# Andy-ckm/K8S-GPU-

Hardware: AMD Instinct MI355X
Metric: p50 reconcile-to-Ready latency (s) + readyReplicas accuracy at replicas=1/2/4/8 (lower is better)
Workload: dtype bf16

## Files before the change

gpupool/ops/probe.py:

```python
from __future__ import annotations

import ctypes
import functools
import json
import threading

from . import lowp, native_path

_lib = None
_lock = threading.Lock()
_count: int | None = None


def lib() -> ctypes.CDLL:
    global _lib
    with _lock:
        if _lib is None:
            l = ctypes.CDLL(native_path("libmi355x_probe.so"))
            l.mi355x_probe_init.restype = ctypes.c_int
            l.mi355x_probe_init.argtypes = [ctypes.c_char_p, ctypes.c_size_t]
            l.mi355x_probe_device_count.restype = ctypes.c_int
            l.mi355x_probe_identify.restype = ctypes.c_void_p
            l.mi355x_probe_identify.argtypes = [ctypes.c_int]
            l.mi355x_probe_run.restype = ctypes.c_void_p
# ... 3 lines not shown
            l.mi355x_probe_peer.argtypes = [ctypes.c_int, ctypes.c_int, ctypes.c_char_p]
            if hasattr(l, "mi355x_probe_peer_ring"):
                l.mi355x_probe_peer_ring.restype = ctypes.c_void_p
                l.mi355x_probe_peer_ring.argtypes = [ctypes.POINTER(ctypes.c_int), ctypes.c_int,
                                                     ctypes.c_char_p]
            l.mi355x_probe_trim.restype = ctypes.c_int
            l.mi355x_probe_trim.argtypes = [ctypes.c_int]
            l.mi355x_probe_hbm_sweep.restype = ctypes.c_void_p
            l.mi355x_probe_hbm_sweep.argtypes = [ctypes.c_int, ctypes.c_char_p]
            l.mi355x_probe_sweep_alloc.restype = ctypes.c_int
            l.mi355x_probe_sweep_alloc.argtypes = [ctypes.c_int, ctypes.c_longlong]
            l.mi355x_probe_sweep_release.restype = ctypes.c_int
            l.mi355x_probe_sweep_release.argtypes = [ctypes.c_int]
            l.mi355x_probe_gemm_bf16.restype = ctypes.c_int
            l.mi355x_probe_gemm_bf16.argtypes = [ctypes.c_int, ctypes.c_void_p, ctypes.c_void_p,
                                                 ctypes.c_void_p, ctypes.c_int, ctypes.c_int,
                                                 ctypes.c_int]
            if hasattr(l, "mi355x_probe_gemm_bf16_opts"):
                l.mi355x_probe_gemm_bf16_opts.restype = ctypes.c_int
                l.mi355x_probe_gemm_bf16_opts.argtypes = [ctypes.c_int, ctypes.c_void_p,
                                                          ctypes.c_void_p, ctypes.c_void_p,
                                                          ctypes.c_int, ctypes.c_int, ctypes.c_int,
                                                          ctypes.c_char_p]
            if hasattr(l, "mi355x_probe_gemm_lowp"):
                l.mi355x_probe_gemm_lowp.restype = ctypes.c_int
                l.mi355x_probe_gemm_lowp.argtypes = [ctypes.c_int, ctypes.c_int] + [ctypes.c_void_p] * 5 + \
                    [ctypes.c_int] * 3 + [ctypes.c_char_p]
            if hasattr(l, "mi355x_probe_host_link"):
                l.mi355x_probe_host_link.restype = ctypes.c_void_p
                l.mi355x_probe_host_link.argtypes = [ctypes.c_int, ctypes.c_char_p, ctypes.c_void_p,
                                                     ctypes.c_size_t]
                l.mi355x_probe_host_link_geometry.restype = None
                l.mi355x_probe_host_link_geometry.argtypes = [ctypes.POINTER(ctypes.c_int)] * 3
            if hasattr(l, "mi355x_probe_lds"):
                l.mi355x_probe_lds.restype = ctypes.c_void_p
                l.mi355x_probe_lds.argtypes = [ctypes.c_int, ctypes.c_char_p, ctypes.c_void_p, ctypes.c_size_t]
            if hasattr(l, "mi355x_probe_abft_check"):
                vp, ull = ctypes.c_void_p, ctypes.c_ulonglong
                l.mi355x_probe_abft_check.restype = ctypes.c_int
                l.mi355x_probe_abft_check.argtypes = [ctypes.c_int, ctypes.c_int] + [vp] * 5 + \
                    [ctypes.c_int] * 3 + [ctypes.c_float, vp, vp, ctypes.c_int, vp, vp, vp]
                l.mi355x_probe_gemm_ref.restype = ctypes.c_int
                l.mi355x_probe_gemm_ref.argtypes = [ctypes.c_int, ctypes.c_int] + [vp] * 5 + [ctypes.c_int] * 3
                l.mi355x_probe_count_diff.restype = ctypes.c_int
                l.mi355x_probe_count_diff.argtypes = [ctypes.c_int, vp, vp, ull, ctypes.POINTER(ull)]
                l.mi355x_probe_gen_operands.restype = ctypes.c_int
                l.mi355x_probe_gen_operands.argtypes = [ctypes.c_int, ctypes.c_int, ctypes.c_uint, ctypes.c_int,
                                                        ull, ull, vp, ctypes.c_size_t, vp, ctypes.c_size_t,
                                                        vp, ctypes.c_size_t]
            _lib = l
    return _lib


def _take(p) -> dict:
    if not p:
        raise RuntimeError("libmi355x_probe returned NULL")
    try:
        return json.loads(ctypes.string_at(p).decode())
    finally:
        lib().mi355x_probe_free(p)


def init() -> int:
    global _count
    if _count is not None:
        return _count
# ... 9 lines not shown
    return _take(lib().mi355x_probe_identify(dev))


def run(dev: int, hbm_bytes: int = 1 << 30, mfma: bool = True, gemm_n: int = 4096,
        patterns: int = 2, gemm_reps: int = 1, gemm_tile: int = 256, mfma_low_precision=(),
        host_link_bytes: int = 0, lds_check: bool = False, **test_hooks: int) -> dict:
    opts = _run_opts(int(hbm_bytes), bool(mfma), int(gemm_n), int(patterns), int(gemm_reps),
                     int(gemm_tile), tuple(sorted((k, int(v)) for k, v in test_hooks.items())),
                     tuple(mfma_low_precision), int(host_link_bytes), bool(lds_check))
    return _take(lib().mi355x_probe_run(dev, opts))


@functools.lru_cache(maxsize=64)
def _run_opts(hbm_bytes: int, mfma: bool, gemm_n: int, patterns: int, gemm_reps: int,
              gemm_tile: int, hooks: tuple, low_precision: tuple = (),
              host_link_bytes: int = 0, lds_check: bool = False) -> bytes:
    opts = {"hbmBytes": hbm_bytes, "mfma": mfma, "gemmN": gemm_n, "patterns": patterns,
            "gemmReps": gemm_reps, "gemmTile": gemm_tile, **dict(hooks)}
    if low_precision:
        opts["mfmaLowPrecision"] = lowp.dtype_mask(low_precision)
    if host_link_bytes > 0:
        opts["hostLinkBytes"] = host_link_bytes
    if lds_check:
        opts["ldsCheck"] = 1
    return json.dumps(opts).encode()


def host_link_geometry() -> dict:
    if not hasattr(lib(), "mi355x_probe_host_link"):
        raise RuntimeError("libmi355x_probe.so predates the host-link check: rebuild it")
    g, t, u = ctypes.c_int(), ctypes.c_int(), ctypes.c_int()
    lib().mi355x_probe_host_link_geometry(ctypes.byref(g), ctypes.byref(t), ctypes.byref(u))
    return {"grid": g.value, "threads": t.value, "unroll": u.value}


def host_link(dev: int, nbytes: int, patterns: int = 2, preload=None, want_bytes: int = 0,
              **hooks: int) -> dict:
    if not hasattr(lib(), "mi355x_probe_host_link"):
        raise RuntimeError("libmi355x_probe.so predates the host-link check: rebuild it")
    opts = {"hostLinkBytes": int(nbytes), "hostLinkPatterns": int(patterns),
            **{k: int(v) for k, v in hooks.items()}}
    buf, n = None, 0
    if preload is not None:
        raw = bytes(preload) if not hasattr(preload, "tobytes") else preload.tobytes()
        n = len(raw)
        buf = ctypes.create_string_buffer(raw, n)
        opts["preload"] = 1
    elif want_bytes > 0:
        n = int(want_bytes)
        buf = ctypes.create_string_buffer(n)
    res = _take(lib().mi355x_probe_host_link(dev, json.dumps(opts).encode(), buf, n))
    if buf is not None and want_bytes > 0 and "bytes" in res:
        res["data"] = buf.raw[:min(int(want_bytes), n, int(res["bytes"]))]
    return res


def lds(dev: int, nbytes: int = 163840, patterns: int = 2, want_stage: int = 0, **hooks: int) -> dict:
    if not hasattr(lib(), "mi355x_probe_lds"):
        raise RuntimeError("libmi355x_probe.so predates the LDS check: rebuild it")
    opts = {"ldsBytes": int(nbytes), "ldsPatterns": int(patterns), **{k: int(v) for k, v in hooks.items()}}
    buf, n = None, 0
    if want_stage:
        opts["ldsDumpStage"] = int(want_stage)
        n = 163840
        buf = ctypes.create_string_buffer(n)
    res = _take(lib().mi355x_probe_lds(dev, json.dumps(opts).encode(), buf, n))
# ... 135 lines not shown
```

native/include/mi355x/probe.h:

```cpp
#ifndef MI355X_PROBE_H_
#define MI355X_PROBE_H_

#include <stddef.h>

#ifdef __cplusplus
extern "C" {
#endif

int mi355x_probe_init(char* err, size_t errlen);
int mi355x_probe_device_count(void);
char* mi355x_probe_identify(int device);
char* mi355x_probe_run(int device, const char* opts_json);
char* mi355x_probe_lds(int device, const char* opts_json, void* image, size_t image_bytes);
char* mi355x_probe_host_link(int device, const char* opts_json, void* io, size_t io_bytes);
void mi355x_probe_host_link_geometry(int* grid, int* threads, int* unroll);
char* mi355x_probe_peer(int src, int dst, const char* opts_json);
char* mi355x_probe_peer_ring(const int* devs, int n, const char* opts_json);
char* mi355x_probe_hbm_sweep(int device, const char* opts_json);
int mi355x_probe_sweep_alloc(int device, long long reserve_bytes);
int mi355x_probe_sweep_release(int device);
int mi355x_probe_gemm_bf16(int device, const void* A, const void* Bt, void* C, int m, int n, int k);
int mi355x_probe_gemm_bf16_opts(int device, const void* A, const void* Bt, void* C, int m, int n, int k,
                                const char* opts_json);
int mi355x_probe_gemm_lowp(int device, int dtype, const void* A, const void* Bt, const void* scaleA,
                           const void* scaleBt, void* C, int m, int n, int k, const char* opts_json);
int mi355x_probe_abft_check(int device, int dtype, const void* A, const void* Bt, const void* scaleA,
                            const void* scaleBt, const void* C, int m, int n, int k, float bound,
                            unsigned int* vectors, unsigned long long* counts, int nfaults,
                            const long long* fault_index, const float* fault_value,
                            unsigned long long* fault_counts);
int mi355x_probe_gemm_ref(int device, int dtype, const void* A, const void* Bt, const void* scaleA,
                          const void* scaleBt, void* R, int m, int n, int k);
int mi355x_probe_count_diff(int device, const float* x, const float* y, unsigned long long count,
                            unsigned long long* bad);
int mi355x_probe_gen_operands(int device, int dtype, unsigned int seed, int span_or_scale_lo,
                              unsigned long long count, unsigned long long nzero, void* operand,
                              size_t operand_bytes, void* scales, size_t scale_bytes, void* zero,
                              size_t zero_bytes);
void mi355x_probe_free(char* p);

#ifdef __cplusplus
}
#endif

#endif
```

native/src/probe/ctx.h:

```cpp
#pragma once

#include <chrono>
#include <cstdio>
#include <cstdlib>
#include <cstring>
#include <mutex>
#include <string>
#include <vector>

#include "arena.h"
#include "options.h"
#include "types.h"

namespace {

struct SweepBuf {
  std::vector<void*> chunks;
  uint64_t span = 0;
  bool empty() const { return chunks.empty(); }
};

struct DeviceCtx {
  hipStream_t stream = nullptr;
  hipStream_t stream2 = nullptr;
  hipEvent_t ev[1 + 2 * kMaxPatterns] = {};
  hipEvent_t gev[3] = {};
  hipDeviceProp_t prop{};
  unsigned long long* host_res = nullptr;
  hipEvent_t lev[lowp::kDtypes][2] = {};
  unsigned long long* host_lowp = nullptr;
  hipStream_t hl_stream = nullptr;
  hipEvent_t hev[1 + 2 * kMaxPatterns] = {};
  void* hl_buf = nullptr;
  void* hl_dev = nullptr;
  uint64_t hl_bytes = 0;
  bool hl_coherent = true;
  unsigned long long* hl_cnt = nullptr;
  unsigned long long* hl_res = nullptr;
  hipEvent_t lds_ev[2] = {};
  unsigned long long* lds_cnt = nullptr;
  unsigned long long* lds_res = nullptr;
  int lds_set = 0;
  bool lds_clean = false;
  uint32_t lds_runs = 0;
  void* lds_dump = nullptr;
  void* arena = nullptr;
  size_t arena_bytes = 0;
  std::chrono::steady_clock::time_point arena_used{};
  SweepBuf sweep;
  unsigned long long* sweep_cnt = nullptr;
  std::chrono::steady_clock::time_point sweep_released{};
  void* peer_send = nullptr;
  void* peer_recv = nullptr;
  uint64_t peer_bytes = 0;
  unsigned long long* peer_cnt = nullptr;
  std::chrono::steady_clock::time_point peer_used{};
  std::string uuid;
  bool ready = false;
};

constexpr std::chrono::seconds kSweepClearGrace{30};
// ... 17 lines not shown
struct DevBuf {
  void* p = nullptr;
  ~DevBuf() {
    if (p) (void)hipFree(p);
  }
};

inline std::string hip_uuid(int dev) {
  hipUUID u{};
  if (hipDeviceGetUuid(&u, dev) != hipSuccess) return "";
  std::string s(u.bytes, u.bytes + 16);
  bool ascii = true;
  for (char c : s) ascii = ascii && ((c >= '0' && c <= '9') || (c >= 'a' && c <= 'f') || (c >= 'A' && c <= 'F'));
  if (ascii) return "GPU-" + s;
  char buf[40];
  std::string hex;
  for (int i = 0; i < 16; ++i) {
    std::snprintf(buf, sizeof buf, "%02x", static_cast<unsigned char>(u.bytes[i]));
    hex += buf;
  }
  return "GPU-" + hex;
}

inline DeviceCtx& ensure_ctx(int dev) {
  PROBE_CHECK(hipSetDevice(dev));
  DeviceCtx& ctx = ctx_of(dev);
  if (ctx.ready) return ctx;
  PROBE_CHECK(hipStreamCreateWithFlags(&ctx.stream, hipStreamNonBlocking));
  PROBE_CHECK(hipStreamCreateWithFlags(&ctx.stream2, hipStreamNonBlocking));
  for (auto& e : ctx.ev) PROBE_CHECK(hipEventCreate(&e));
  for (auto& e : ctx.gev) PROBE_CHECK(hipEventCreate(&e));
  PROBE_CHECK(hipGetDeviceProperties(&ctx.prop, dev));
  PROBE_CHECK(hipHostMalloc(reinterpret_cast<void**>(&ctx.host_res), kResSlots * sizeof(unsigned long long)));
  ctx.uuid = hip_uuid(dev);
  ctx.ready = true;
  return ctx;
}

}
```

native/src/probe/hbm.h:

```cpp
#pragma once

#include <algorithm>
#include <cstdint>

#include "options.h"
#include "report.h"
#include "types.h"

namespace {

__host__ __device__ __forceinline__ uint32_t pattern_word(uint64_t idx, uint32_t seed) {
  uint32_t x = static_cast<uint32_t>(idx) * 0x9E3779B1u ^ static_cast<uint32_t>(idx >> 32) * 0x85EBCA77u;
  x ^= seed;
  x ^= x >> 15;
  x *= 0x2C1B3C6Du;
  x ^= x >> 12;
  return x;
}

template <int kPat>
__host__ __device__ __forceinline__ u32x4 pattern16(uint64_t i16, uint32_t seed, uint32_t flip) {
  u32x4 v;
  if constexpr (kPat == 0) {
    uint64_t w = i16 * 4;
    v.x = pattern_word(w, seed) ^ flip;
    v.y = pattern_word(w + 1, seed) ^ flip;
    v.z = pattern_word(w + 2, seed) ^ flip;
    v.w = pattern_word(w + 3, seed) ^ flip;
  } else {
    uint32_t h = (static_cast<uint32_t>(i16) ^ seed) * 0x9E3779B1u;
    h ^= __builtin_rotateleft32(static_cast<uint32_t>(i16 >> 32), 7);
    h ^= h >> 15;
    v.x = h ^ flip;
    v.y = __builtin_rotateleft32(h, 8) ^ 0xA5A5A5A5u ^ flip;
    v.z = __builtin_rotateleft32(h, 16) ^ 0x3C96C396u ^ flip;
    v.w = __builtin_rotateleft32(h, 24) ^ 0x5A0FF05Au ^ flip;
  }
  return v;
}
__device__ __forceinline__ uint64_t umin64(uint64_t a, uint64_t b) { return a < b ? a : b; }

constexpr int kHbmThreads = 256;
constexpr int kHbmUnroll = 4;

constexpr uint64_t kHbmTile = static_cast<uint64_t>(kHbmThreads) * kHbmUnroll;

__device__ __forceinline__ void reset_pairs(unsigned long long* __restrict__ cnt, int nreset) {
  if (blockIdx.x == 0 && static_cast<int>(threadIdx.x) < 2 * nreset)
    cnt[threadIdx.x] = (threadIdx.x & 1) ? ~0ull : 0ull;
}

template <int kPat = kHbmPattern, int kLayout = 0>
__global__ __launch_bounds__(kHbmThreads) void hbm_fill(u32x4* __restrict__ p, uint64_t n16,
                                                        uint32_t seed, uint32_t flip,
                                                        unsigned long long* __restrict__ reset, int nreset) {
  reset_pairs(reset, nreset);
  const uint64_t stride = static_cast<uint64_t>(gridDim.x) * kHbmThreads;
  if constexpr (kLayout == 1) {
    const uint64_t tiles = n16 / kHbmTile;
    for (uint64_t t = blockIdx.x; t < tiles; t += gridDim.x) {
      const uint64_t base = t * kHbmTile + threadIdx.x;
#pragma unroll
      for (int u = 0; u < kHbmUnroll; ++u) {
        const uint64_t j = base + static_cast<uint64_t>(u) * kHbmThreads;
        __builtin_nontemporal_store(pattern16<kPat>(j, seed, flip), &p[j]);
      }
    }
    for (uint64_t i = tiles * kHbmTile + static_cast<uint64_t>(blockIdx.x) * kHbmThreads + threadIdx.x; i < n16;
         i += stride)
      __builtin_nontemporal_store(pattern16<kPat>(i, seed, flip), &p[i]);
    return;
  }
  uint64_t i = static_cast<uint64_t>(blockIdx.x) * kHbmThreads + threadIdx.x;
  for (; i + (kHbmUnroll - 1) * stride < n16; i += kHbmUnroll * stride) {
#pragma unroll
    for (int u = 0; u < kHbmUnroll; ++u) {
      uint64_t j = i + u * stride;
      __builtin_nontemporal_store(pattern16<kPat>(j, seed, flip), &p[j]);
    }
  }
  for (; i < n16; i += stride) __builtin_nontemporal_store(pattern16<kPat>(i, seed, flip), &p[i]);
}

__device__ __forceinline__ uint32_t mismatches16(u32x4 v, u32x4 e) {
  return __builtin_popcount(v.x ^ e.x) + __builtin_popcount(v.y ^ e.y) +
         __builtin_popcount(v.z ^ e.z) + __builtin_popcount(v.w ^ e.w);
}

template <int kPat = kHbmPattern, int kLayout = 0>
__global__ __launch_bounds__(kHbmThreads) void hbm_verify(const u32x4* __restrict__ p, uint64_t n16,
                                                          uint32_t seed, uint32_t flip,
                                                          unsigned long long* __restrict__ bad_bits,
                                                          unsigned long long* __restrict__ first_bad) {
  const uint64_t stride = static_cast<uint64_t>(gridDim.x) * kHbmThreads;
  uint32_t bad = 0;
  uint64_t first = ~0ull;
  auto check = [&](u32x4 v, uint64_t j) {
    uint32_t m = mismatches16(v, pattern16<kPat>(j, seed, flip));
    if (m) {
      bad += m;
      first = umin64(first, j);
    }
  };
  if constexpr (kLayout == 1) {
    const uint64_t tiles = n16 / kHbmTile;
    for (uint64_t t = blockIdx.x; t < tiles; t += gridDim.x) {
      const uint64_t base = t * kHbmTile + threadIdx.x;
      u32x4 v[kHbmUnroll];
#pragma unroll
      for (int u = 0; u < kHbmUnroll; ++u) v[u] = __builtin_nontemporal_load(&p[base + static_cast<uint64_t>(u) * kHbmThreads]);
#pragma unroll
      for (int u = 0; u < kHbmUnroll; ++u) check(v[u], base + static_cast<uint64_t>(u) * kHbmThreads);
    }
    for (uint64_t i = tiles * kHbmTile + static_cast<uint64_t>(blockIdx.x) * kHbmThreads + threadIdx.x; i < n16;
         i += stride)
      check(__builtin_nontemporal_load(&p[i]), i);
  } else {
    uint64_t i = static_cast<uint64_t>(blockIdx.x) * kHbmThreads + threadIdx.x;
    for (; i + (kHbmUnroll - 1) * stride < n16; i += kHbmUnroll * stride) {
      u32x4 v[kHbmUnroll];
#pragma unroll
      for (int u = 0; u < kHbmUnroll; ++u) v[u] = __builtin_nontemporal_load(&p[i + u * stride]);
#pragma unroll
      for (int u = 0; u < kHbmUnroll; ++u) check(v[u], i + u * stride);
    }
    for (; i < n16; i += stride) check(__builtin_nontemporal_load(&p[i]), i);
  }
#pragma unroll
  for (int off = 32; off > 0; off >>= 1) {
    bad += __shfl_xor(bad, off, 64);
    first = umin64(first, static_cast<uint64_t>(__shfl_xor(static_cast<unsigned long long>(first), off, 64)));
  }
  if ((threadIdx.x & 63) == 0 && bad) {
    atomicAdd(bad_bits, static_cast<unsigned long long>(bad));
    atomicMin(first_bad, static_cast<unsigned long long>(first));
  }
}
__global__ void inject_bit_flips(unsigned int* __restrict__ p, uint64_t nwords, int count) {
  const uint64_t stride = nwords / static_cast<uint64_t>(count + 1);
  for (int i = threadIdx.x; i < count; i += blockDim.x) p[static_cast<uint64_t>(i + 1) * stride] ^= 1u << (i % 32);
}

static_assert(2 * kMaxPatterns <= kHbmThreads, "hbm_fill resets the HBM pairs from one block");

inline int hbm_grid(int cus, long long per_cu, uint64_t n16) {
  return static_cast<int>(std::min<uint64_t>(static_cast<uint64_t>(cus) * static_cast<uint64_t>(per_cu),
                                             (n16 + kHbmThreads - 1) / kHbmThreads));
}

inline void memset_pairs(hipStream_t s, unsigned long long* cnt, int zero_words, int npairs) {
  PROBE_CHECK(hipMemsetAsync(cnt, 0, zero_words * sizeof(unsigned long long), s));
  for (int pi = 0; pi < npairs; ++pi)
    PROBE_CHECK(hipMemsetAsync(cnt + 2 * pi + 1, 0xFF, sizeof(unsigned long long), s));
}

struct PatternPass {
  hipStream_t s = nullptr;
  u32x4* buf = nullptr;
  uint64_t n16 = 0;
  uint32_t seed = 0;
  int fill_grid = 1, verify_grid = 1;
  bool cheap = kHbmPattern == 1, tiled = false;

  static uint32_t flip_of(int pi) { return (pi & 1) ? 0xFFFFFFFFu : 0u; }

  void fill(int pi, unsigned long long* reset = nullptr, int nreset = 0) const {
    const dim3 grid(fill_grid), block(kHbmThreads);
    if (tiled) hipLaunchKernelGGL((hbm_fill<1, 1>), grid, block, 0, s, buf, n16, seed, flip_of(pi), reset, nreset);
    else if (cheap) hipLaunchKernelGGL(hbm_fill<1>, grid, block, 0, s, buf, n16, seed, flip_of(pi), reset, nreset);
    else hipLaunchKernelGGL(hbm_fill<0>, grid, block, 0, s, buf, n16, seed, flip_of(pi), reset, nreset);
  }

  void verify(int pi, unsigned long long* pair) const {
    const dim3 grid(verify_grid), block(kHbmThreads);
    const u32x4* p = buf;
    if (tiled) hipLaunchKernelGGL((hbm_verify<1, 1>), grid, block, 0, s, p, n16, seed, flip_of(pi), pair, pair + 1);
    else if (cheap) hipLaunchKernelGGL(hbm_verify<1>, grid, block, 0, s, p, n16, seed, flip_of(pi), pair, pair + 1);
    else hipLaunchKernelGGL(hbm_verify<0>, grid, block, 0, s, p, n16, seed, flip_of(pi), pair, pair + 1);
  }

  void inject_flips(int count) const {
    hipLaunchKernelGGL(inject_bit_flips, dim3(1), dim3(256), 0, s, reinterpret_cast<unsigned int*>(buf), n16 * 4, count);
  }
  void inject_flip_at(uint64_t chunk) const {
    hipLaunchKernelGGL(inject_bit_flips, dim3(1), dim3(256), 0, s, reinterpret_cast<unsigned int*>(buf + chunk),
                       uint64_t{0}, 1);
  }
};

inline void fold_pairs(const unsigned long long* pairs, int patterns, HbmResult* r) {
  for (int pi = 0; pi < patterns; ++pi) {
    r->bad_bits += pairs[2 * pi];
    r->first_bad = std::min(r->first_bad, pairs[2 * pi + 1]);
  }
}

inline HbmResult fold_passes(const hipEvent_t* ev, const unsigned long long* pairs, int patterns, uint64_t n16) {
  HbmResult r;
  r.n16 = n16;
  r.patterns = patterns;
  for (int pi = 0; pi < patterns; ++pi) {
    float w, rd;
    PROBE_CHECK(hipEventElapsedTime(&w, ev[2 * pi], ev[1 + 2 * pi]));
    PROBE_CHECK(hipEventElapsedTime(&rd, ev[1 + 2 * pi], ev[2 + 2 * pi]));
    r.write_ms += w;
    r.read_ms += rd;
  }
  fold_pairs(pairs, patterns, &r);
  return r;
}

// ... 2 lines not shown
```

native/src/probe/options.h:

```cpp
#pragma once

#include <algorithm>
#include <cstdint>
#include <cstdlib>
#include <cstring>
#include <stdexcept>
#include <string>

namespace {

inline long long opt_int(const char* json, const char* key, long long def) {
  if (!json) return def;
  std::string pat = std::string("\"") + key + "\"";
  const char* p = std::strstr(json, pat.c_str());
  if (!p) return def;
  p = std::strchr(p + pat.size(), ':');
  if (!p) return def;
  ++p;
  while (*p == ' ') ++p;
  if (std::strncmp(p, "true", 4) == 0) return 1;
  if (std::strncmp(p, "false", 5) == 0) return 0;
  return std::strtoll(p, nullptr, 10);
}

inline bool opt_bool(const char* json, const char* key, bool def) { return opt_int(json, key, def) != 0; }

constexpr long long kMaxPatterns = 4;

constexpr int kHbmPattern = 1;
constexpr int kHbmLayout = 0;
constexpr long long kHbmFillBlocksPerCU = 1, kHbmVerifyBlocksPerCU = 3;

constexpr int kGemmGroupM = 4;
constexpr int kGemmPipe = 2;

struct GemmVariant {
  int tile = 256;
  int pipe = kGemmPipe;
  bool prio = false;
  bool vec_c = false;
};

struct GemmOptions {
  GemmVariant variant;
  int group_m = kGemmGroupM;
  bool poison_c = false;
  static GemmOptions parse(const char* json) {
    GemmOptions o;
    o.variant.tile = static_cast<int>(opt_int(json, "gemmTile", 256));
    o.variant.pipe = static_cast<int>(opt_int(json, "gemmPipe", kGemmPipe));
    o.variant.prio = opt_bool(json, "gemmPrio", false);
    o.variant.vec_c = opt_bool(json, "gemmVecC", false);
    o.group_m = static_cast<int>(opt_int(json, "gemmGroupM", kGemmGroupM));
    o.poison_c = opt_bool(json, "poisonC", false);
    return o;
  }
};

namespace lowp {
enum Dtype { kFp8 = 0, kMxFp8 = 1, kMxFp4 = 2, kDtypes = 3 };
constexpr const char* kNames[kDtypes] = {"fp8", "mxfp8", "mxfp4"};
}

// ... 72 lines not shown
    pl.n16 = static_cast<uint32_t>(bytes / 16);
    pl.patterns = static_cast<int>(std::min(kMaxPatterns, std::max(1LL, opt_int(json, "ldsPatterns", 2))));
    const long long salt = opt_int(json, "ldsSalt", -1);
    pl.salt_given = salt >= 0;
    pl.salt = pl.salt_given ? static_cast<uint32_t>(salt) : 0u;
    pl.seed = 0x4C445300u + static_cast<uint32_t>(dev);
    pl.blocks_per_cu =
        static_cast<int>(std::min<long long>(kMaxBlocksPerCU, std::max(1LL, opt_int(json, "ldsBlocksPerCU", kBlocksPerCU))));
    pl.flip_byte = opt_int(json, "injectLdsFlipAtByte", -1);
    pl.fault_xcc = static_cast<int>(opt_int(json, "injectLdsFaultXcc", -1));
    pl.skip_chunk = opt_int(json, "injectLdsSkipChunk", -1);
    const long long stage = opt_int(json, "ldsDumpStage", 0);
    pl.dump_stage = stage >= 1 && stage <= 3 ? static_cast<int>(stage) : 0;
    return pl;
  }
};

}

struct FaultAt {
  long long row = -1, col = -1;
  long long index(int n) const {
    const long long r = row == -1 ? n / 3 : row, c = col == -1 ? n / 5 : col;
    if (r < 0 || r >= n || c < 0 || c >= n) return -1;
    return r * n + c;
  }
};

struct ProbeOptions {
  uint64_t hbm_bytes = 1ull << 30;
  int patterns = 2;
  bool cheap_pattern = true;
  bool tiled = false;
  long long fill_blocks_per_cu = kHbmFillBlocksPerCU;
  long long verify_blocks_per_cu = kHbmVerifyBlocksPerCU;
  int inject_flips = 0;
  long long inject_chunk = -1;
  bool mfma = true;
  int gemm_n = 4096;
  GemmOptions gemm;
  int reps = 1;
  int inject_gemm = 0;
  FaultAt inject_gemm_at;
  int census_fault_xcc = -1;
  bool require_all_cus = true;
  bool cu_keys = false;
  int lowp_mask = 0;
  int inject_lowp = 0;
  int lowp_census_fault_xcc = -1;
  bool overlap = true;
  int hbm_first = 1;
  bool zero_in_kernel = true;
  bool keep_arena = true;
  hostlink::Plan host_link;
  bool host_link_on_mfma_stream = false;
  lds::Plan lds;
  bool lds_first = lds::kFirst == 1;

  static ProbeOptions parse(const char* json, int dev = 0) {
    ProbeOptions o;
    o.hbm_bytes = static_cast<uint64_t>(opt_int(json, "hbmBytes", 1LL << 30));
    o.patterns = static_cast<int>(std::min(kMaxPatterns, std::max(1LL, opt_int(json, "patterns", 2))));
    o.cheap_pattern = opt_int(json, "hbmPattern", kHbmPattern) == 1;
    o.tiled = o.cheap_pattern && opt_int(json, "hbmLayout", kHbmLayout) == 1;
    o.fill_blocks_per_cu =
        std::max(1LL, opt_int(json, "hbmFillBlocksPerCU", opt_int(json, "hbmBlocksPerCU", kHbmFillBlocksPerCU)));
    o.verify_blocks_per_cu =
        std::max(1LL, opt_int(json, "hbmVerifyBlocksPerCU", opt_int(json, "hbmBlocksPerCU", kHbmVerifyBlocksPerCU)));
    o.inject_flips = static_cast<int>(std::min(4096LL, std::max(0LL, opt_int(json, "injectBitFlips", 0))));
    o.inject_chunk = opt_int(json, "injectFlipAtChunk", -1);
    o.mfma = opt_bool(json, "mfma", true);
    o.gemm_n = std::max(256, (static_cast<int>(opt_int(json, "gemmN", 4096)) / 256) * 256);
    o.gemm = GemmOptions::parse(json);
    o.gemm.variant.tile = o.gemm.variant.tile != 128 ? 256 : 128;
    o.reps = opt_int(json, "gemmSkip", 0) ? 0 : static_cast<int>(std::max(1LL, opt_int(json, "gemmReps", 1)));
    o.inject_gemm = static_cast<int>(opt_int(json, "injectGemmFault", 0));
    o.inject_gemm_at.row = opt_int(json, "injectGemmFaultRow", -1);
    o.inject_gemm_at.col = opt_int(json, "injectGemmFaultCol", -1);
    o.census_fault_xcc = static_cast<int>(opt_int(json, "injectCensusFaultXcc", -1));
    o.require_all_cus = opt_bool(json, "requireAllCUs", true);
    o.cu_keys = opt_bool(json, "cuKeys", false);
    o.lowp_mask = o.mfma ? static_cast<int>(opt_int(json, "mfmaLowPrecision", 0)) & ((1 << lowp::kDtypes) - 1) : 0;
    o.inject_lowp = static_cast<int>(opt_int(json, "injectLowpFault", 0));
    o.lowp_census_fault_xcc = static_cast<int>(opt_int(json, "injectLowpCensusFaultXcc", -1));
    o.overlap = opt_bool(json, "overlap", true);
    o.hbm_first = static_cast<int>(opt_int(json, "hbmFirst", 1));
    o.zero_in_kernel = opt_bool(json, "zeroInKernel", true);
    o.keep_arena = opt_bool(json, "keepArena", true);
    const uint64_t hl_bytes = static_cast<uint64_t>(std::max(0LL, opt_int(json, "hostLinkBytes", 0)));
    if (hl_bytes > hostlink::kMaxBytes) throw std::invalid_argument("hostLinkBytes above 4 GiB");
    if (hl_bytes) {
      o.host_link = hostlink::Plan::parse(json, dev, hl_bytes);
      o.host_link_on_mfma_stream = o.overlap && opt_int(json, "hostLinkStream", 0) == 1;
    }
    if (opt_bool(json, "ldsCheck", false)) {
      o.lds = lds::Plan::parse(json, dev);
      o.lds.dump_stage = 0;
      o.lds_first = opt_int(json, "ldsFirst", lds::kFirst) == 1;
    }
    return o;
  }
};

struct HostLinkOptions {
  bool preload = false;
  uint64_t bytes = 0;
  static HostLinkOptions parse(const char* json) {
    HostLinkOptions o;
    o.preload = opt_bool(json, "preload", false);
    o.bytes = static_cast<uint64_t>(std::max(0LL, opt_int(json, "hostLinkBytes", 0)));
    return o;
  }
};

inline uint64_t peer_bytes(const char* json, long long def) {
  return static_cast<uint64_t>(std::max(1LL << 20, opt_int(json, "bytes", def)));
}

struct SweepOptions {
  uint64_t bytes = 16ull << 30;
  uint64_t reserve = 4ull << 30;
// ... 16 lines not shown
```

native/src/probe/probe.hip:

```cpp
#include <hip/hip_runtime.h>

#include <algorithm>
#include <chrono>
#include <cstdlib>
#include <cstring>
#include <mutex>
#include <string>
#include <vector>

#include "mi355x/probe.h"

#include "arena.h"
#include "ctx.h"
#include "hbm.h"
#include "hostlink.h"
#include "lds.h"
#include "lowp.h"
#include "mfma_phase.h"
#include "options.h"
#include "peer.h"
#include "report.h"
#include "sweep.h"
#include "types.h"

// ... 44 lines not shown
  memset_pairs(s, cnt, kResSlots, o.patterns);
  if (o.overlap) {
    PROBE_CHECK(hipEventRecord(ctx.gev[2], s));
    PROBE_CHECK(hipStreamWaitEvent(s2, ctx.gev[2], 0));
  }
}

lowp::Phase lowp_phase(DeviceCtx& ctx, const ProbeOptions& o, char* base, const ArenaLayout& lay) {
  lowp::Phase lp;
  lp.mask = o.lowp_mask;
  lp.region = base + lay.lowp_region;
  lp.cnt = reinterpret_cast<unsigned long long*>(base + lay.lowp_cnt);
  lp.host = ctx.host_lowp;
  lp.ev = ctx.lev;
  lp.gemm_n = o.gemm_n;
  lp.cus = ctx.prop.multiProcessorCount;
  lp.inject_mask = o.inject_lowp;
  lp.inject_at = o.inject_gemm_at.index(o.gemm_n);
  lp.census_fault_xcc = o.lowp_census_fault_xcc;
  lp.poison_c = o.gemm.poison_c;
  return lp;
}

PatternPass hbm_pass(DeviceCtx& ctx, const ProbeOptions& o, int dev, char* base, const ArenaLayout& lay, uint64_t n16) {
  PatternPass pass;
  pass.s = ctx.stream;
  pass.buf = reinterpret_cast<u32x4*>(base + lay.hbm);
  pass.n16 = n16;
  pass.seed = 0xA5A50000u + static_cast<uint32_t>(dev);
  pass.fill_grid = hbm_grid(ctx.prop.multiProcessorCount, o.fill_blocks_per_cu, n16);
  pass.verify_grid = hbm_grid(ctx.prop.multiProcessorCount, o.verify_blocks_per_cu, n16);
  pass.cheap = o.cheap_pattern;
  pass.tiled = o.tiled;
  return pass;
}

template <class F>
void enqueue_hbm(DeviceCtx& ctx, const PatternPass& pass, const ProbeOptions& o, unsigned long long* cnt,
                 F&& after_first_fill) {
  PROBE_CHECK(hipEventRecord(ctx.ev[0], pass.s));
  for (int pi = 0; pi < o.patterns; ++pi) {
    unsigned long long* reset = o.zero_in_kernel && pi == 0 ? cnt : nullptr;
    pass.fill(pi, reset, reset ? o.patterns : 0);
    PROBE_CHECK(hipEventRecord(ctx.ev[1 + 2 * pi], pass.s));
    if (pi == 0) {
      after_first_fill();
      if (o.inject_flips > 0) pass.inject_flips(o.inject_flips);
      if (o.inject_chunk >= 0 && static_cast<uint64_t>(o.inject_chunk) < pass.n16)
        pass.inject_flip_at(static_cast<uint64_t>(o.inject_chunk));
    }
    pass.verify(pi, cnt + 2 * pi);
    PROBE_CHECK(hipEventRecord(ctx.ev[2 + 2 * pi], pass.s));
  }
  PROBE_CHECK(hipGetLastError());
  PROBE_CHECK(hipMemcpyAsync(ctx.host_res, cnt, 2 * o.patterns * sizeof(unsigned long long), hipMemcpyDeviceToHost, pass.s));
}

std::string run_probe(int dev, const char* opts) {
  const ProbeOptions o = ProbeOptions::parse(opts, dev);
  auto t0 = std::chrono::steady_clock::now();
  DeviceCtx& ctx = ensure_ctx(dev);
  if (o.lowp_mask) ensure_lowp(ctx);
  hostlink::Plan hl = o.host_link;
  hipStream_t s = ctx.stream, s2 = o.overlap ? ctx.stream2 : s, hl_s = s;
  if (hl.n16) {
    hl.alloc_ms = hostlink::ensure(ctx, hl.n16 * 16, hl.coherent);
// ... 8 lines not shown

  auto t_alloc = std::chrono::steady_clock::now();
  const uint64_t n16 = o.hbm_bytes / 16;
  const ArenaLayout lay = ArenaLayout::make(n16, o.gemm_n, o.mfma, o.lowp_mask);
  DevBuf transient;
  char* base = acquire_arena(ctx, lay.need, o.keep_arena, &transient, &t.arena_reused);
  auto* cnt = reinterpret_cast<unsigned long long*>(base + lay.cnt);
  t.alloc_ms = ms_since(t_alloc);

  auto t_run = std::chrono::steady_clock::now();
  reset_counters(ctx, o, cnt, s, s2);
  const lowp::Phase lp = lowp_phase(ctx, o, base, lay);
  bool lds_pending = ld.n16 != 0;
  auto enqueue_lds = [&](bool here) {
    if (!lds_pending || !here) return;
    lds::launch(ctx, s2, ld);
    lds_pending = false;
  };
  auto enqueue_mfma = [&](int when) {
    if (!o.mfma || o.hbm_first != when) return;
    enqueue_lds(o.overlap && o.lds_first);
    launch_mfma_phase(base, lay, o, ctx, s2);
    lowp::launch(s2, lp);
    enqueue_lds(o.overlap);
  };
  const PatternPass pass = hbm_pass(ctx, o, dev, base, lay, n16);
  enqueue_mfma(0);
  enqueue_hbm(ctx, pass, o, cnt, [&] { enqueue_mfma(2); });
  enqueue_mfma(1);
  enqueue_lds(true);
  if (hl.n16) hostlink::launch(ctx, hl_s, hl);
  t.launch_ms = ms_since(t_run);

  PROBE_CHECK(hipStreamSynchronize(s));
  t.hbm_wall_ms = ms_since(t_run);
  rep.mfma.enabled = o.mfma;
  rep.mfma.n = o.gemm_n;
  rep.mfma.tile = o.gemm.variant.tile;
  rep.mfma.pipe = o.gemm.variant.tile == 256 ? o.gemm.variant.pipe : 0;
  if (o.mfma) {
    PROBE_CHECK(hipStreamSynchronize(s2));
    finish_mfma(o, ctx, &rep.mfma, &rep.cus);
  }
  rep.has_lds = ld.n16 != 0;
  if (ld.n16) {
    if (!o.mfma && s2 != s) PROBE_CHECK(hipStreamSynchronize(s2));
    rep.lds = lds::finish(ctx, ld, o.require_all_cus);
  }
  rep.lowp = lowp::finish(lp, o.require_all_cus);
  t.mfma_wall_ms = o.mfma ? ms_since(t_run) : 0.0;
  rep.has_host_link = hl.n16 != 0;
  if (hl.n16) {
    if (hl_s != s && !(hl_s == ctx.stream2 && o.mfma)) PROBE_CHECK(hipStreamSynchronize(hl_s));
    rep.host_link = hostlink::finish(ctx, hl);
  }
  rep.hbm = fold_passes(ctx.ev, ctx.host_res, o.patterns, n16);
  auto t_free = std::chrono::steady_clock::now();
  if (transient.p) {
    (void)hipFree(transient.p);
    transient.p = nullptr;
  }
  t.free_ms = ms_since(t_free);
  rep.total_ms = ms_since(t0);

  const auto t_report = std::chrono::steady_clock::now();
  rep.dev = dev;
  rep.uuid = ctx.uuid;
  rep.arch = ctx.prop.gcnArchName;
  std::string out = probe_report_open(rep);
  out += ",\"reportMs\":" + jnum(ms_since(t_report)) + "}";
  return out;
}

template <class F>
char* guarded(const std::string& head, F&& body) {
  try {
    return dup(body());
  } catch (const std::exception& e) {
    (void)hipGetLastError();
    return dup(error_report(head, e.what()));
  }
}

// ... 362 lines not shown
    need = count * 2;
  } else {
    if (count % (32 / lowp::bits_of(dtype)) || nzero || zero || span_or_scale_lo < -126 || span_or_scale_lo > 126) return -2;
    need = count * lowp::bits_of(dtype) / 8;
  }
  if (operand_bytes < need || (has_scales ? (!scales || scale_bytes < count / 32) : scales != nullptr)) return -2;
  if (zero ? zero_bytes < nzero * 4 : nzero > 0) return -2;
  std::lock_guard<std::mutex> g(device_mutex(dev));
  return guarded_status([&] {
    PROBE_CHECK(hipSetDevice(dev));
    DevBuf dop, dsc, dz;
    auto filled = [](DevBuf& d, size_t bytes) {
      PROBE_CHECK(hipMalloc(&d.p, std::max<size_t>(bytes, 16)));
      PROBE_CHECK(hipMemset(d.p, 0xFF, std::max<size_t>(bytes, 16)));
    };
    filled(dop, operand_bytes);
    if (has_scales) filled(dsc, scale_bytes);
    if (zero) filled(dz, zero_bytes);
    launch_generator(nullptr, dtype, dop.p, count, static_cast<uint8_t*>(dsc.p), seed, span_or_scale_lo,
                     static_cast<uint32_t*>(dz.p), nzero);
    PROBE_CHECK(hipGetLastError());
    PROBE_CHECK(hipMemcpy(operand, dop.p, operand_bytes, hipMemcpyDeviceToHost));
    if (has_scales && scale_bytes) PROBE_CHECK(hipMemcpy(scales, dsc.p, scale_bytes, hipMemcpyDeviceToHost));
    if (zero && zero_bytes) PROBE_CHECK(hipMemcpy(zero, dz.p, zero_bytes, hipMemcpyDeviceToHost));
  });
}

void mi355x_probe_host_link_geometry(int* grid, int* threads, int* unroll) {
  if (grid) *grid = hostlink::kGrid;
  if (threads) *threads = hostlink::kThreads;
  if (unroll) *unroll = hostlink::kUnroll;
}

char* mi355x_probe_host_link(int dev, const char* opts_json, void* io, size_t io_bytes) {
  if (!device_ok(dev)) return bad_device();
  const HostLinkOptions o = HostLinkOptions::parse(opts_json);
  if (o.preload && !io) return dup(error_report("", "preload needs a caller buffer"));
  ProbeActive active;
  std::lock_guard<std::mutex> g(device_mutex(dev));
  return guarded(device_head(dev), [&] {
    DeviceCtx& ctx = ensure_ctx(dev);
    const uint64_t bytes = o.preload ? static_cast<uint64_t>(io_bytes) : o.bytes;
    if (bytes < 16 || bytes > hostlink::kMaxBytes) throw ProbeError("host-link size outside [16 B, 4 GiB]");
    hostlink::Plan pl = hostlink::Plan::parse(opts_json, dev, bytes);
    if (o.preload) {
      pl.preload = true;
      pl.patterns = 1;
    }
    pl.alloc_ms = hostlink::ensure(ctx, pl.n16 * 16, pl.coherent);
    if (o.preload) std::memcpy(ctx.hl_buf, io, pl.n16 * 16);
    hostlink::launch(ctx, ctx.stream, pl);
    PROBE_CHECK(hipStreamSynchronize(ctx.stream));
    const HostLinkResult r = hostlink::finish(ctx, pl);
    if (io) std::memcpy(io, ctx.hl_buf, std::min<uint64_t>(io_bytes, pl.n16 * 16));
    return "{" + device_head(dev) + ",\"passed\":" + jbool(r.ok()) + "," + host_link_block(r).substr(1);
  });
}

int mi355x_probe_gemm_bf16(int dev, const void* A, const void* Bt, void* C, int m, int n, int k) {
  return mi355x_probe_gemm_bf16_opts(dev, A, Bt, C, m, n, k, nullptr);
}

char* mi355x_probe_lds(int dev, const char* opts_json, void* image, size_t image_bytes) {
  if (!device_ok(dev)) return bad_device();
  ProbeActive active;
  std::lock_guard<std::mutex> g(device_mutex(dev));
// ... 19 lines not shown
```

Before: 0.005100.

## Add atomic work-claiming tail layout to HBM fill/verify and fold side streams first

Adds a new HBM layout, made the default, where each block strides through a static head region and then takes row units of the remaining tail through a global atomic counter. The aim is to balance load across blocks and stop the slowest CU from setting the finish time of the fill and verify passes. It also changes the host ordering so results from the side streams (MFMA, LDS) are synchronized and folded before the wait on the main HBM stream, overlapping that host work. The costs are per-block atomics, per-pass counter resets that chain kernels through a `next` pointer, and added geometry bookkeeping with bounds checks in the tail.

```diff
diff --git a/gpupool/ops/probe.py b/gpupool/ops/probe.py
--- a/gpupool/ops/probe.py
+++ b/gpupool/ops/probe.py
@@ -59,6 +59,11 @@
                                                      ctypes.c_size_t]
                 l.mi355x_probe_host_link_geometry.restype = None
                 l.mi355x_probe_host_link_geometry.argtypes = [ctypes.POINTER(ctypes.c_int)] * 3
+            if hasattr(l, "mi355x_probe_hbm_claim_geometry"):
+                ullp = ctypes.POINTER(ctypes.c_ulonglong)
+                l.mi355x_probe_hbm_claim_geometry.restype = ctypes.c_int
+                l.mi355x_probe_hbm_claim_geometry.argtypes = [ctypes.c_int, ctypes.c_ulonglong, ctypes.c_int, ullp, ullp,
+                                                              ctypes.POINTER(ctypes.c_uint), ullp]
             if hasattr(l, "mi355x_probe_lds"):
                 l.mi355x_probe_lds.restype = ctypes.c_void_p
                 l.mi355x_probe_lds.argtypes = [ctypes.c_int, ctypes.c_char_p, ctypes.c_void_p, ctypes.c_size_t]
@@ -134,6 +139,17 @@
     g, t, u = ctypes.c_int(), ctypes.c_int(), ctypes.c_int()
     lib().mi355x_probe_host_link_geometry(ctypes.byref(g), ctypes.byref(t), ctypes.byref(u))
     return {"grid": g.value, "threads": t.value, "unroll": u.value}
+
+
+def hbm_claim_geometry(dev: int, nbytes: int, verify: bool = False) -> dict:
+    if not hasattr(lib(), "mi355x_probe_hbm_claim_geometry"):
+        raise RuntimeError("libmi355x_probe.so predates the claimed HBM layout: rebuild it")
+    head, units, width, rows = ctypes.c_ulonglong(), ctypes.c_ulonglong(), ctypes.c_ulonglong(), ctypes.c_uint()
+    rc = lib().mi355x_probe_hbm_claim_geometry(dev, int(nbytes), int(bool(verify)), ctypes.byref(head),
+                                               ctypes.byref(units), ctypes.byref(rows), ctypes.byref(width))
+    if rc != 0:
+        raise RuntimeError(f"mi355x_probe_hbm_claim_geometry failed (rc={rc})")
+    return {"head": head.value, "units": units.value, "unitRows": rows.value, "rowWidth": width.value}
 
 
 def host_link(dev: int, nbytes: int, patterns: int = 2, preload=None, want_bytes: int = 0,
diff --git a/native/include/mi355x/probe.h b/native/include/mi355x/probe.h
--- a/native/include/mi355x/probe.h
+++ b/native/include/mi355x/probe.h
@@ -14,6 +14,9 @@
 char* mi355x_probe_lds(int device, const char* opts_json, void* image, size_t image_bytes);
 char* mi355x_probe_host_link(int device, const char* opts_json, void* io, size_t io_bytes);
 void mi355x_probe_host_link_geometry(int* grid, int* threads, int* unroll);
+int mi355x_probe_hbm_claim_geometry(int device, unsigned long long bytes, int verify, unsigned long long* head,
+                                    unsigned long long* units, unsigned int* unit_rows,
+                                    unsigned long long* row_width);
 char* mi355x_probe_peer(int src, int dst, const char* opts_json);
 char* mi355x_probe_peer_ring(const int* devs, int n, const char* opts_json);
 char* mi355x_probe_hbm_sweep(int device, const char* opts_json);
diff --git a/native/src/probe/ctx.h b/native/src/probe/ctx.h
--- a/native/src/probe/ctx.h
+++ b/native/src/probe/ctx.h
@@ -27,6 +27,8 @@
   hipEvent_t gev[3] = {};
   hipDeviceProp_t prop{};
   unsigned long long* host_res = nullptr;
+  unsigned int* hbm_claims = nullptr;
+  bool hbm_claims_clean = false;
   hipEvent_t lev[lowp::kDtypes][2] = {};
   unsigned long long* host_lowp = nullptr;
   hipStream_t hl_stream = nullptr;
@@ -110,6 +112,9 @@
   for (auto& e : ctx.gev) PROBE_CHECK(hipEventCreate(&e));
   PROBE_CHECK(hipGetDeviceProperties(&ctx.prop, dev));
   PROBE_CHECK(hipHostMalloc(reinterpret_cast<void**>(&ctx.host_res), kResSlots * sizeof(unsigned long long)));
+  PROBE_CHECK(hipMalloc(reinterpret_cast<void**>(&ctx.hbm_claims), 2 * kMaxPatterns * sizeof(unsigned int)));
+  PROBE_CHECK(hipMemsetAsync(ctx.hbm_claims, 0, 2 * kMaxPatterns * sizeof(unsigned int), ctx.stream));
+  ctx.hbm_claims_clean = true;
   ctx.uuid = hip_uuid(dev);
   ctx.ready = true;
   return ctx;
diff --git a/native/src/probe/hbm.h b/native/src/probe/hbm.h
--- a/native/src/probe/hbm.h
+++ b/native/src/probe/hbm.h
@@ -3,6 +3,7 @@
 #include <algorithm>
 #include <cstdint>
 
+#include "hbm_claims.h"
 #include "options.h"
 #include "report.h"
 #include "types.h"
@@ -44,6 +45,41 @@
 constexpr int kHbmUnroll = 4;
 
 constexpr uint64_t kHbmTile = static_cast<uint64_t>(kHbmThreads) * kHbmUnroll;
+static_assert(kHbmThreads == kHbmClaimColumn && kHbmUnroll == kHbmClaimUnroll, "hbm_claims.h describes these kernels");
+
+struct HbmClaims {
+  unsigned int* counter = nullptr;
+  unsigned int* next = nullptr;
+  uint64_t head = 0, units = 0, tail_rows = 0;
+  uint32_t rows = 0;
+};
+
+template <class Four, class One>
+__device__ __forceinline__ void hbm_claimed_tail(const HbmClaims& c, uint64_t n16, uint64_t width, Four&& four, One&& one) {
+  __shared__ unsigned int handed[2];
+  HbmClaimGeometry g;
+  g.n16 = n16;
+  g.width = width;
+  g.head = c.head;
+  g.units = c.units;
+  g.tail_rows = c.tail_rows;
+  g.rows = c.rows;
+  if (threadIdx.x == 0) handed[0] = atomicInc(c.counter, ~0u);
+  __syncthreads();
+  unsigned int cur = handed[0], claimed = 0;
+  for (int slot = 1; cur < g.units; slot ^= 1) {
+    if (threadIdx.x == 0) claimed = atomicInc(c.counter, ~0u);
+    const HbmClaimUnit u = hbm_claim_unit(g, cur);
+    uint64_t i = u.first + threadIdx.x;
+    uint32_t r = 0;
+    for (; hbm_claim_rows_whole(g, u, r); r += kHbmUnroll, i += kHbmUnroll * width) four(i);
+    for (; r < u.rows; ++r, i += width)
+      if (i < n16) one(i);
+    if (threadIdx.x == 0) handed[slot] = claimed;
+    __syncthreads();
+    cur = handed[slot];
+  }
+}
 
 __device__ __forceinline__ void reset_pairs(unsigned long long* __restrict__ cnt, int nreset) {
   if (blockIdx.x == 0 && static_cast<int>(threadIdx.x) < 2 * nreset)
@@ -53,9 +89,24 @@
 template <int kPat = kHbmPattern, int kLayout = 0>
 __global__ __launch_bounds__(kHbmThreads) void hbm_fill(u32x4* __restrict__ p, uint64_t n16,
                                                         uint32_t seed, uint32_t flip,
-                                                        unsigned long long* __restrict__ reset, int nreset) {
+                                                        unsigned long long* __restrict__ reset, int nreset,
+                                                        const HbmClaims c) {
   reset_pairs(reset, nreset);
   const uint64_t stride = static_cast<uint64_t>(gridDim.x) * kHbmThreads;
+  if constexpr (kLayout == 2) {
+    if (blockIdx.x == 0 && threadIdx.x == 0) *c.next = 0;
+    auto four = [&](uint64_t i) {
+#pragma unroll
+      for (int u = 0; u < kHbmUnroll; ++u) {
+        const uint64_t j = i + u * stride;
+        __builtin_nontemporal_store(pattern16<kPat>(j, seed, flip), &p[j]);
+      }
+    };
+    for (uint64_t i = static_cast<uint64_t>(blockIdx.x) * kHbmThreads + threadIdx.x; i < c.head; i += kHbmUnroll * stride) four(i);
+    hbm_claimed_tail(c, n16, stride, four,
+                     [&](uint64_t j) { __builtin_nontemporal_store(pattern16<kPat>(j, seed, flip), &p[j]); });
+    return;
+  }
   if constexpr (kLayout == 1) {
     const uint64_t tiles = n16 / kHbmTile;
     for (uint64_t t = blockIdx.x; t < tiles; t += gridDim.x) {
@@ -91,7 +142,8 @@
 __global__ __launch_bounds__(kHbmThreads) void hbm_verify(const u32x4* __restrict__ p, uint64_t n16,
                                                           uint32_t seed, uint32_t flip,
                                                           unsigned long long* __restrict__ bad_bits,
-                                                          unsigned long long* __restrict__ first_bad) {
+                                                          unsigned long long* __restrict__ first_bad,
+                                                          const HbmClaims c) {
   const uint64_t stride = static_cast<uint64_t>(gridDim.x) * kHbmThreads;
   uint32_t bad = 0;
   uint64_t first = ~0ull;
@@ -102,7 +154,18 @@
       first = umin64(first, j);
     }
   };
-  if constexpr (kLayout == 1) {
+  if constexpr (kLayout == 2) {
+    if (blockIdx.x == 0 && threadIdx.x == 0) *c.next = 0;
+    auto four = [&](uint64_t i) {
+      u32x4 v[kHbmUnroll];
+#pragma unroll
+      for (int u = 0; u < kHbmUnroll; ++u) v[u] = __builtin_nontemporal_load(&p[i + u * stride]);
+#pragma unroll
+      for (int u = 0; u < kHbmUnroll; ++u) check(v[u], i + u * stride);
+    };
+    for (uint64_t i = static_cast<uint64_t>(blockIdx.x) * kHbmThreads + threadIdx.x; i < c.head; i += kHbmUnroll * stride) four(i);
+    hbm_claimed_tail(c, n16, stride, four, [&](uint64_t j) { check(__builtin_nontemporal_load(&p[j]), j); });
+  } else if constexpr (kLayout == 1) {
     const uint64_t tiles = n16 / kHbmTile;
     for (uint64_t t = blockIdx.x; t < tiles; t += gridDim.x) {
       const uint64_t base = t * kHbmTile + threadIdx.x;
@@ -161,22 +224,46 @@
   uint32_t seed = 0;
   int fill_grid = 1, verify_grid = 1;
   bool cheap = kHbmPattern == 1, tiled = false;
+  unsigned int* claims = nullptr;
+  int patterns = 0;
+  uint32_t claim_rows = kHbmClaimRows, claim_tail_shift = kHbmClaimTailShift, claim_verify_tail_shift = kHbmClaimVerifyTailShift;
 
   static uint32_t flip_of(int pi) { return (pi & 1) ? 0xFFFFFFFFu : 0u; }
+
+  HbmClaims claims_of(int k, int grid) const {
+    const HbmClaimGeometry g =
+        hbm_claim_geometry(n16, static_cast<uint32_t>(grid), claim_rows, (k & 1) ? claim_verify_tail_shift : claim_tail_shift);
+    if (g.units + static_cast<uint64_t>(grid) > 0x7FFFFFFFull) throw ProbeError("hbmLayout 2: too many units for this region");
+    HbmClaims c;
+    c.counter = claims + k;
+    c.next = claims + (k + 1) % (2 * patterns);
+    c.head = g.head;
+    c.units = g.units;
+    c.tail_rows = g.tail_rows;
+    c.rows = g.rows;
+    return c;
+  }
 
   void fill(int pi, unsigned long long* reset = nullptr, int nreset = 0) const {
     const dim3 grid(fill_grid), block(kHbmThreads);
-    if (tiled) hipLaunchKernelGGL((hbm_fill<1, 1>), grid, block, 0, s, buf, n16, seed, flip_of(pi), reset, nreset);
-    else if (cheap) hipLaunchKernelGGL(hbm_fill<1>, grid, block, 0, s, buf, n16, seed, flip_of(pi), reset, nreset);
-    else hipLaunchKernelGGL(hbm_fill<0>, grid, block, 0, s, buf, n16, seed, flip_of(pi), reset, nreset);
+    const HbmClaims none;
+    if (claims)
+      hipLaunchKernelGGL((hbm_fill<1, 2>), grid, block, 0, s, buf, n16, seed, flip_of(pi), reset, nreset, claims_of(2 * pi, fill_grid));
+    else if (tiled) hipLaunchKernelGGL((hbm_fill<1, 1>), grid, block, 0, s, buf, n16, seed, flip_of(pi), reset, nreset, none);
+    else if (cheap) hipLaunchKernelGGL(hbm_fill<1>, grid, block, 0, s, buf, n16, seed, flip_of(pi), reset, nreset, none);
+    else hipLaunchKernelGGL(hbm_fill<0>, grid, block, 0, s, buf, n16, seed, flip_of(pi), reset, nreset, none);
   }
 
   void verify(int pi, unsigned long long* pair) const {
     const dim3 grid(verify_grid), block(kHbmThreads);
     const u32x4* p = buf;
-    if (tiled) hipLaunchKernelGGL((hbm_verify<1, 1>), grid, block, 0, s, p, n16, seed, flip_of(pi), pair, pair + 1);
-    else if (cheap) hipLaunchKernelGGL(hbm_verify<1>, grid, block, 0, s, p, n16, seed, flip_of(pi), pair, pair + 1);
-    else hipLaunchKernelGGL(hbm_verify<0>, grid, block, 0, s, p, n16, seed, flip_of(pi), pair, pair + 1);
+    const HbmClaims none;
+    if (claims)
+      hipLaunchKernelGGL((hbm_verify<1, 2>), grid, block, 0, s, p, n16, seed, flip_of(pi), pair, pair + 1,
+                         claims_of(2 * pi + 1, verify_grid));
+    else if (tiled) hipLaunchKernelGGL((hbm_verify<1, 1>), grid, block, 0, s, p, n16, seed, flip_of(pi), pair, pair + 1, none);
+    else if (cheap) hipLaunchKernelGGL(hbm_verify<1>, grid, block, 0, s, p, n16, seed, flip_of(pi), pair, pair + 1, none);
+    else hipLaunchKernelGGL(hbm_verify<0>, grid, block, 0, s, p, n16, seed, flip_of(pi), pair, pair + 1, none);
   }
 
   void inject_flips(int count) const {
diff --git a/native/src/probe/hbm_claims.h b/native/src/probe/hbm_claims.h
--- /dev/null
+++ b/native/src/probe/hbm_claims.h
@@ -0,0 +1,55 @@
+#pragma once
+
+#include <cstdint>
+
+#if defined(__HIPCC__)
+#define HBM_CLAIMS_FN __host__ __device__ __forceinline__
+#else
+#define HBM_CLAIMS_FN inline
+#endif
+
+constexpr uint32_t kHbmClaimColumn = 256;
+constexpr uint32_t kHbmClaimUnroll = 4;
+
+struct HbmClaimGeometry {
+  uint64_t n16 = 0;
+  uint64_t width = 0;
+  uint64_t head = 0;
+  uint64_t units = 0;
+  uint64_t tail_rows = 0;
+  uint32_t rows = 0;
+};
+
+HBM_CLAIMS_FN HbmClaimGeometry hbm_claim_geometry(uint64_t n16, uint32_t grid, uint32_t rows, uint32_t tail_shift) {
+  HbmClaimGeometry g;
+  g.n16 = n16;
+  g.width = static_cast<uint64_t>(grid) * kHbmClaimColumn;
+  g.rows = rows;
+  if (grid == 0 || rows == 0) return g;
+  const uint64_t quantum = kHbmClaimUnroll * g.width;
+  g.head = (n16 - (n16 >> tail_shift)) / quantum * quantum;
+  g.tail_rows = (n16 - g.head + g.width - 1) / g.width;
+  g.units = (g.tail_rows + rows - 1) / rows * grid;
+  return g;
+}
+
+struct HbmClaimUnit {
+  uint64_t first = 0;
+  uint32_t rows = 0;
+};
+
+HBM_CLAIMS_FN HbmClaimUnit hbm_claim_unit(const HbmClaimGeometry& g, uint64_t claim) {
+  HbmClaimUnit u;
+  if (claim >= g.units) return u;
+  const uint32_t grid = static_cast<uint32_t>(g.width / kHbmClaimColumn), c = static_cast<uint32_t>(claim);
+  const uint64_t row = static_cast<uint64_t>(c / grid) * g.rows, col = static_cast<uint64_t>(c % grid) * kHbmClaimColumn;
+  u.first = g.head + row * g.width + col;
+  const uint64_t left = g.tail_rows - row;
+  u.rows = left < g.rows ? static_cast<uint32_t>(left) : g.rows;
+  if (row + u.rows == g.tail_rows && g.head + (g.tail_rows - 1) * g.width + col >= g.n16) --u.rows;
+  return u;
+}
+
+HBM_CLAIMS_FN bool hbm_claim_rows_whole(const HbmClaimGeometry& g, const HbmClaimUnit& u, uint32_t r) {
+  return r + kHbmClaimUnroll <= u.rows && u.first + (r + kHbmClaimUnroll - 1) * g.width + kHbmClaimColumn <= g.n16;
+}
diff --git a/native/src/probe/options.h b/native/src/probe/options.h
--- a/native/src/probe/options.h
+++ b/native/src/probe/options.h
@@ -28,7 +28,8 @@
 constexpr long long kMaxPatterns = 4;
 
 constexpr int kHbmPattern = 1;
-constexpr int kHbmLayout = 0;
+constexpr int kHbmLayout = 2;
+constexpr int kHbmClaimRows = 32, kHbmClaimTailShift = 1, kHbmClaimVerifyTailShift = 63;
 constexpr long long kHbmFillBlocksPerCU = 1, kHbmVerifyBlocksPerCU = 3;
 
 constexpr int kGemmGroupM = 4;
@@ -167,6 +168,10 @@
   int patterns = 2;
   bool cheap_pattern = true;
   bool tiled = false;
+  int hbm_layout = kHbmLayout;
+  int claim_rows = kHbmClaimRows;
+  int claim_tail_shift = kHbmClaimTailShift;
+  int claim_verify_tail_shift = kHbmClaimVerifyTailShift;
   long long fill_blocks_per_cu = kHbmFillBlocksPerCU;
   long long verify_blocks_per_cu = kHbmVerifyBlocksPerCU;
   int inject_flips = 0;
@@ -187,6 +192,7 @@
   int hbm_first = 1;
   bool zero_in_kernel = true;
   bool keep_arena = true;
+  bool side_fold_first = true;
   hostlink::Plan host_link;
   bool host_link_on_mfma_stream = false;
   lds::Plan lds;
@@ -197,7 +203,13 @@
     o.hbm_bytes = static_cast<uint64_t>(opt_int(json, "hbmBytes", 1LL << 30));
     o.patterns = static_cast<int>(std::min(kMaxPatterns, std::max(1LL, opt_int(json, "patterns", 2))));
     o.cheap_pattern = opt_int(json, "hbmPattern", kHbmPattern) == 1;
-    o.tiled = o.cheap_pattern && opt_int(json, "hbmLayout", kHbmLayout) == 1;
+    const long long layout = opt_int(json, "hbmLayout", kHbmLayout);
+    o.hbm_layout = o.cheap_pattern && (layout == 1 || layout == 2) ? static_cast<int>(layout) : 0;
+    o.tiled = o.hbm_layout == 1;
+    o.claim_rows = static_cast<int>(std::min(1024LL, std::max(4LL, opt_int(json, "hbmClaimRows", kHbmClaimRows))) / 4 * 4);
+    o.claim_tail_shift = static_cast<int>(std::min(63LL, std::max(0LL, opt_int(json, "hbmClaimTailShift", kHbmClaimTailShift))));
+    o.claim_verify_tail_shift =
+        static_cast<int>(std::min(63LL, std::max(0LL, opt_int(json, "hbmClaimVerifyTailShift", kHbmClaimVerifyTailShift))));
     o.fill_blocks_per_cu =
         std::max(1LL, opt_int(json, "hbmFillBlocksPerCU", opt_int(json, "hbmBlocksPerCU", kHbmFillBlocksPerCU)));
     o.verify_blocks_per_cu =
@@ -222,6 +234,7 @@
     o.hbm_first = static_cast<int>(opt_int(json, "hbmFirst", 1));
     o.zero_in_kernel = opt_bool(json, "zeroInKernel", true);
     o.keep_arena = opt_bool(json, "keepArena", true);
+    o.side_fold_first = opt_bool(json, "sideFoldFirst", true);
     const uint64_t hl_bytes = static_cast<uint64_t>(std::max(0LL, opt_int(json, "hostLinkBytes", 0)));
     if (hl_bytes > hostlink::kMaxBytes) throw std::invalid_argument("hostLinkBytes above 4 GiB");
     if (hl_bytes) {
diff --git a/native/src/probe/probe.hip b/native/src/probe/probe.hip
--- a/native/src/probe/probe.hip
+++ b/native/src/probe/probe.hip
@@ -100,6 +100,16 @@
   pass.verify_grid = hbm_grid(ctx.prop.multiProcessorCount, o.verify_blocks_per_cu, n16);
   pass.cheap = o.cheap_pattern;
   pass.tiled = o.tiled;
+  if (o.hbm_layout == 2) {
+    if (!ctx.hbm_claims_clean)
+      PROBE_CHECK(hipMemsetAsync(ctx.hbm_claims, 0, 2 * kMaxPatterns * sizeof(unsigned int), ctx.stream));
+    ctx.hbm_claims_clean = false;
+    pass.claims = ctx.hbm_claims;
+    pass.patterns = o.patterns;
+    pass.claim_rows = static_cast<uint32_t>(o.claim_rows);
+    pass.claim_tail_shift = static_cast<uint32_t>(o.claim_tail_shift);
+    pass.claim_verify_tail_shift = static_cast<uint32_t>(o.claim_verify_tail_shift);
+  }
   return pass;
 }
 
@@ -174,23 +184,29 @@
   if (hl.n16) hostlink::launch(ctx, hl_s, hl);
   t.launch_ms = ms_since(t_run);
 
-  PROBE_CHECK(hipStreamSynchronize(s));
-  t.hbm_wall_ms = ms_since(t_run);
   rep.mfma.enabled = o.mfma;
   rep.mfma.n = o.gemm_n;
   rep.mfma.tile = o.gemm.variant.tile;
   rep.mfma.pipe = o.gemm.variant.tile == 256 ? o.gemm.variant.pipe : 0;
-  if (o.mfma) {
-    PROBE_CHECK(hipStreamSynchronize(s2));
-    finish_mfma(o, ctx, &rep.mfma, &rep.cus);
-  }
   rep.has_lds = ld.n16 != 0;
-  if (ld.n16) {
-    if (!o.mfma && s2 != s) PROBE_CHECK(hipStreamSynchronize(s2));
-    rep.lds = lds::finish(ctx, ld, o.require_all_cus);
-  }
-  rep.lowp = lowp::finish(lp, o.require_all_cus);
-  t.mfma_wall_ms = o.mfma ? ms_since(t_run) : 0.0;
+  auto fold_side = [&] {
+    if (o.mfma) {
+      PROBE_CHECK(hipStreamSynchronize(s2));
+      finish_mfma(o, ctx, &rep.mfma, &rep.cus);
+    }
+    if (ld.n16) {
+      if (!o.mfma && s2 != s) PROBE_CHECK(hipStreamSynchronize(s2));
+      rep.lds = lds::finish(ctx, ld, o.require_all_cus);
+    }
+    rep.lowp = lowp::finish(lp, o.require_all_cus);
+    t.mfma_wall_ms = o.mfma ? ms_since(t_run) : 0.0;
+  };
+  const bool side_first = s2 != s && o.side_fold_first;
+  if (side_first) fold_side();
+  PROBE_CHECK(hipStreamSynchronize(s));
+  if (pass.claims) ctx.hbm_claims_clean = true;
+  t.hbm_wall_ms = ms_since(t_run);
+  if (!side_first) fold_side();
   rep.has_host_link = hl.n16 != 0;
   if (hl.n16) {
     if (hl_s != s && !(hl_s == ctx.stream2 && o.mfma)) PROBE_CHECK(hipStreamSynchronize(hl_s));
@@ -619,6 +635,23 @@
   if (unroll) *unroll = hostlink::kUnroll;
 }
 
+int mi355x_probe_hbm_claim_geometry(int dev, unsigned long long bytes, int verify, unsigned long long* head,
+                                    unsigned long long* units, unsigned int* unit_rows, unsigned long long* row_width) {
+  if (!device_ok(dev)) return -1;
+  std::lock_guard<std::mutex> g(device_mutex(dev));
+  return guarded_status([&] {
+    const DeviceCtx& ctx = ensure_ctx(dev);
+    const uint64_t n16 = bytes / 16;
+    const int grid = hbm_grid(ctx.prop.multiProcessorCount, verify ? kHbmVerifyBlocksPerCU : kHbmFillBlocksPerCU, n16);
+    const HbmClaimGeometry geo = hbm_claim_geometry(n16, static_cast<uint32_t>(grid), kHbmClaimRows,
+                                                    verify ? kHbmClaimVerifyTailShift : kHbmClaimTailShift);
+    if (head) *head = geo.head;
+    if (units) *units = geo.units;
+    if (unit_rows) *unit_rows = geo.rows;
+    if (row_width) *row_width = geo.width;
+  });
+}
+
 char* mi355x_probe_host_link(int dev, const char* opts_json, void* io, size_t io_bytes) {
   if (!device_ok(dev)) return bad_device();
   const HostLinkOptions o = HostLinkOptions::parse(opts_json);
```

Result: no change. 0.005100 (+0.0%).
